# modelstreaming/ams

Hardware: AMD Instinct MI355X
Metric: frames/sec student infer (DeeplabV3+MobileNetV2, 512x1024) + distill-steps/sec (higher is better)
Workload: dtype f32 (2xfp16 split products)

## Files before the change

ams_amd/csrc/k_head.hip:

```cpp
#include "head_common.hpp"

namespace ams {

template <int KMAX>
__global__ __launch_bounds__(256) void upsample_argmax_kernel(const float* __restrict__ logits, HeadGeom g, ClassTable ct,
                                                              const uint8_t* __restrict__ teacher,
                                                              int32_t* __restrict__ labels,
                                                              unsigned long long* __restrict__ conf, double* __restrict__ loss) {
    __shared__ int s_conf[kMaxK * kMaxK];
    __shared__ double s_loss[4];
    __shared__ int s_cnt[4];
    const bool metric = teacher != nullptr;
    if (metric)
        for (int e = threadIdx.x; e < g.K * g.K; e += blockDim.x) s_conf[e] = 0;
    const int b = blockIdx.z;
    if (g.per_frame && metric) { conf += (size_t)b * g.K * g.K; loss += 2 * b; }
    const int x = blockIdx.x * blockDim.x + threadIdx.x;
    if (metric) __syncthreads();
    double my_loss = 0.0;
    int my_cnt = 0;
    int x0 = 0, x1 = 0; float tx = 0.f;
    if (x < g.W) src_tap(x, g.sx, g.w, x0, x1, tx);
    const float* base = logits + (int64_t)b * g.h * g.w * g.ld;
    const int band = (g.H + (int)gridDim.y - 1) / (int)gridDim.y;
    const int ybeg = blockIdx.y * band, yend = ybeg + band < g.H ? ybeg + band : g.H;
    constexpr int KR = KMAX > 0 ? KMAX : 1;
    float top[KR], bot[KR];
    int cur_y0 = -1;
    for (int y = ybeg; y < yend; ++y) {
        if (x >= g.W) break;
        int y0, y1; float ty;
        src_tap(y, g.sy, g.h, y0, y1, ty);
        const float* ptl = base + ((int64_t)y0 * g.w + x0) * g.ld;
        const float* ptr = base + ((int64_t)y0 * g.w + x1) * g.ld;
        const float* pbl = base + ((int64_t)y1 * g.w + x0) * g.ld;
        const float* pbr = base + ((int64_t)y1 * g.w + x1) * g.ld;
        if (KMAX > 0 && y0 != cur_y0) {
            cur_y0 = y0;
#pragma unroll
            for (int k = 0; k < KR; ++k) {
                const int c = ct.idx[k < g.K ? k : 0];
                top[k] = __fadd_rn(ptl[c], __fmul_rn(__fsub_rn(ptr[c], ptl[c]), tx));
                bot[k] = __fadd_rn(pbl[c], __fmul_rn(__fsub_rn(pbr[c], pbl[c]), tx));
            }
        }
        const int64_t pix = ((int64_t)b * g.H + y) * g.W + x;
        int target = -1;
        if (metric) target = ct.lut[teacher[pix]];
        float best = 0.f, zt = 0.f, zmax = 0.f, ssum = 0.f;
        int arg = 0;
        auto visit = [&](int k, float v) {
            if (k == 0 || v > best) { best = v; arg = k; }
            if (target >= 0) {
                if (k == 0) { zmax = v; ssum = 1.f; }
                else if (v > zmax) { ssum = ssum * __expf(zmax - v) + 1.f; zmax = v; }
                else ssum += __expf(v - zmax);
                if (k == target) zt = v;
            }
        };
        if (KMAX > 0) {
#pragma unroll
            for (int k = 0; k < KR; ++k)
                if (k < g.K) visit(k, __fadd_rn(top[k], __fmul_rn(__fsub_rn(bot[k], top[k]), ty)));
        } else {
            for (int k = 0; k < g.K; ++k) {
                const int c = ct.idx[k];
                visit(k, bilerp(ptl[c], ptr[c], pbl[c], pbr[c], tx, ty));
            }
        }
        if (labels) { if (g.labels_u8) reinterpret_cast<uint8_t*>(labels)[pix] = (uint8_t)arg; else labels[pix] = arg; }
        if (target >= 0) {
            my_loss += rint((double)((zmax + __logf(ssum)) - zt) * 1048576.0);
            my_cnt += 1;
            atomicAdd(&s_conf[target * g.K + arg], 1);
        }
    }
    if (!metric) return;
    my_loss = wave_sum(my_loss);
    my_cnt = (int)wave_sum((float)my_cnt);
    const int wave = threadIdx.x >> 6;
    if ((threadIdx.x & 63) == 0) { s_loss[wave] = my_loss; s_cnt[wave] = my_cnt; }
    __syncthreads();
    for (int e = threadIdx.x; e < g.K * g.K; e += blockDim.x)
        if (s_conf[e]) atomicAdd(&conf[e], (unsigned long long)s_conf[e]);
    if (threadIdx.x == 0) {
        const int nw = (blockDim.x + 63) >> 6;
        double ls = 0; int cn = 0;
        for (int i = 0; i < nw; ++i) { ls += s_loss[i]; cn += s_cnt[i]; }
        if (cn) { atomicAdd(&loss[0], ls * (1.0 / 1048576.0)); atomicAdd(&loss[1], (double)cn); }
    }
}

int launch_upsample_argmax(const HeadCall& c, int32_t* labels, int64_t* conf, double* loss, hipStream_t st, int per_frame, int labels_u8) {
    ClassTable ct;
    HeadGeom g;
    if (int rc = head_call_check("upsample_argmax", c, &ct, &g)) return rc;
    AMS_REQUIRE(c.teacher == nullptr || (conf != nullptr && loss != nullptr), "upsample_argmax: metrics need conf and loss buffers");
    AMS_REQUIRE(c.logits, "upsample_argmax: null pointer");
    const int nm = per_frame ? c.B : 1;
    if (c.teacher) {
        AMS_CHECK_HIP(hipMemsetAsync(conf, 0, sizeof(int64_t) * c.K * c.K * nm, st));
        AMS_CHECK_HIP(hipMemsetAsync(loss, 0, sizeof(double) * 2 * nm, st));
    }
    g.per_frame = per_frame;
    g.labels_u8 = labels_u8;
    note_kernel("upsample_argmax_kernel");
    const dim3 grid = head_band_grid(c.B, c.H, c.W);
    if (c.K <= 8)
        hipLaunchKernelGGL(upsample_argmax_kernel<8>, grid, dim3(256), 0, st, c.logits, g, ct, c.teacher, labels, (unsigned long long*)conf, loss);
    else
        hipLaunchKernelGGL(upsample_argmax_kernel<0>, grid, dim3(256), 0, st, c.logits, g, ct, c.teacher, labels, (unsigned long long*)conf, loss);
    AMS_CHECK_LAUNCH();
    return AMS_OK;
}

template <int KMAX>
__global__ __launch_bounds__(256) void ce_grad_kernel(const float* __restrict__ logits, HeadGeom g, ClassTable ct,
                                                      const uint8_t* __restrict__ teacher,
                                                      const double* __restrict__ loss_and_count, float* __restrict__ dlogits,
                                                      int ldd, float empty_val) {
    __shared__ float s_part[4][KMAX];
    const int j = blockIdx.x, i = blockIdx.y, b = blockIdx.z;
    const double nvalid = loss_and_count[1];
    const float inv_n = nvalid > 0.5 ? (float)(1.0 / nvalid) : 0.f;
    const float ry = g.sy > 0.f ? 1.f / g.sy : 0.f, rx = g.sx > 0.f ? 1.f / g.sx : 0.f;
    int ya = g.sy > 0.f ? (int)floorf((i - 1) * ry) - 1 : 0, yb = g.sy > 0.f ? (int)ceilf((i + 1) * ry) + 1 : g.H - 1;
    int xa = g.sx > 0.f ? (int)floorf((j - 1) * rx) - 1 : 0, xb = g.sx > 0.f ? (int)ceilf((j + 1) * rx) + 1 : g.W - 1;
    ya = ya < 0 ? 0 : ya; xa = xa < 0 ? 0 : xa;
    yb = yb > g.H - 1 ? g.H - 1 : yb; xb = xb > g.W - 1 ? g.W - 1 : xb;
    const int ny = yb - ya + 1, nx = xb - xa + 1;
    float acc[KMAX];
#pragma unroll
    for (int k = 0; k < KMAX; ++k) acc[k] = 0.f;
    const float* base = logits + (int64_t)b * g.h * g.w * g.ld;
    for (int p = threadIdx.x; p < ny * nx; p += blockDim.x) {
        const int y = ya + p / nx, x = xa + p % nx;
        int y0, y1, x0, x1; float ty, tx;
        src_tap(y, g.sy, g.h, y0, y1, ty);
        src_tap(x, g.sx, g.w, x0, x1, tx);
        float wy = 0.f, wx = 0.f;
        if (y0 == i) wy += 1.f - ty;
        if (y1 == i) wy += ty;
        if (x0 == j) wx += 1.f - tx;
        if (x1 == j) wx += tx;
        const float wgt = wy * wx;
        if (wgt == 0.f) continue;
        const int target = ct.lut[teacher[((int64_t)b * g.H + y) * g.W + x]];
        if (target < 0) continue;
        const float* ptl = base + ((int64_t)y0 * g.w + x0) * g.ld;
        const float* ptr = base + ((int64_t)y0 * g.w + x1) * g.ld;
        const float* pbl = base + ((int64_t)y1 * g.w + x0) * g.ld;
        const float* pbr = base + ((int64_t)y1 * g.w + x1) * g.ld;
        float z[KMAX];
        float zmax = -3.0e38f;
#pragma unroll
        for (int k = 0; k < KMAX; ++k) {
            if (k < g.K) {
                const int c = ct.idx[k];
                z[k] = bilerp(ptl[c], ptr[c], pbl[c], pbr[c], tx, ty);
                zmax = fmaxf(zmax, z[k]);
            } else z[k] = 0.f;
        }
        float ssum = 0.f;
#pragma unroll
        for (int k = 0; k < KMAX; ++k)
            if (k < g.K) { z[k] = __expf(z[k] - zmax); ssum += z[k]; }
        const float f = wgt * inv_n, rs = 1.f / ssum;
#pragma unroll
        for (int k = 0; k < KMAX; ++k)
            if (k < g.K) acc[k] += f * (z[k] * rs - (k == target ? 1.f : 0.f));
    }
    const int wave = threadIdx.x >> 6, lane = threadIdx.x & 63;
#pragma unroll
    for (int k = 0; k < KMAX; ++k) {
        const float s = wave_sum(acc[k]);
        if (lane == 0) s_part[wave][k] = s;
    }
    __syncthreads();
    float* out = dlogits + (((int64_t)b * g.h + i) * g.w + j) * ldd;
    for (int c = threadIdx.x; c < ldd; c += blockDim.x) {
        float v = 0.f;
        if (c < 256) {
            const int k = ct.lut[c];
            if (k >= 0) v = (s_part[0][k] + s_part[1][k]) + (s_part[2][k] + s_part[3][k]);
            if (k >= 0 && !(nvalid > 0.5)) v = empty_val;
        }
        out[c] = v;
    }
}

int launch_ce_grad(const HeadCall& c, const double* loss_and_count, float* dlogits, int ldd, hipStream_t st, float empty_val) {
    ClassTable ct;
    HeadGeom g;
    if (int rc = head_call_check("ce_grad", c, &ct, &g)) return rc;
    AMS_REQUIRE(ldd >= c.NC && ldd <= 256, "ce_grad: ldd=%d must hold %d classes", ldd, c.NC);
    AMS_REQUIRE(c.logits && c.teacher && loss_and_count && dlogits, "ce_grad: null pointer");
    const dim3 grid(c.w, c.h, c.B);
    note_kernel(c.K <= 8 ? "ce_grad_kernel<8>" : c.K <= 20 ? "ce_grad_kernel<20>" : "ce_grad_kernel<32>");
    if (c.K <= 8)
        hipLaunchKernelGGL(ce_grad_kernel<8>, grid, dim3(256), 0, st, c.logits, g, ct, c.teacher, loss_and_count, dlogits, ldd, empty_val);
    else if (c.K <= 20)
        hipLaunchKernelGGL(ce_grad_kernel<20>, grid, dim3(256), 0, st, c.logits, g, ct, c.teacher, loss_and_count, dlogits, ldd, empty_val);
    else
        hipLaunchKernelGGL(ce_grad_kernel<32>, grid, dim3(256), 0, st, c.logits, g, ct, c.teacher, loss_and_count, dlogits, ldd, empty_val);
    AMS_CHECK_LAUNCH();
    return AMS_OK;
}

constexpr int kCeCB = 10;

template <int KMAX, bool SOFT = false, int KD = 0, bool WT = false>
__global__ __launch_bounds__(192) __attribute__((amdgpu_waves_per_eu(KD != 0 && KMAX == 20 ? 2 : 0)))
void ce_loss_grad_kernel(const float* __restrict__ logits, HeadGeom g, ClassTable ct,
                                                           const uint8_t* __restrict__ teacher, double* __restrict__ loss,
                                                           float* __restrict__ partT, float* __restrict__ partB, SoftTeacher sft, KdParams kd,
                                                           std::conditional_t<WT, LossWeights, NoLossWeights> lw) {
    static_assert(KD == 0 || SOFT, "the KD forms read the teacher logits");
    __shared__ float s_val[192][2 * KMAX + 1];
    __shared__ float s_wx[192][2];
    __shared__ int s_x0[192];
    __shared__ double s_loss[3];
    __shared__ int s_cnt[3];
    __shared__ double s_w[WT ? 3 : 1];
    const int b = blockIdx.z, i0 = blockIdx.y, j_lo = blockIdx.x * kCeCB;
    const int i1 = i0 + 1 < g.h ? i0 + 1 : g.h - 1;
    int ybeg, yend;
    {
        const float inv = g.sy > 0.f ? 1.f / g.sy : 0.f;
        int y = g.sy > 0.f ? (int)(i0 * inv) - 2 : 0;
        if (y < 0) y = 0;
        while (y < g.H && (int)floorf(__fmul_rn((float)y, g.sy)) < i0) ++y;
        ybeg = y;
        while (y < g.H && (int)floorf(__fmul_rn((float)y, g.sy)) == i0) ++y;
        yend = y;
    }
    int xbeg;
    {
        const float inv = g.sx > 0.f ? 1.f / g.sx : 0.f;
        const int jl = j_lo - 1 < 0 ? 0 : j_lo - 1;
        int x = g.sx > 0.f ? (int)(jl * inv) - 2 : 0;
        if (x < 0) x = 0;
        while (x < g.W && (int)floorf(__fmul_rn((float)x, g.sx)) < jl) ++x;
        xbeg = x;
    }
    const int x = xbeg + threadIdx.x;
    int x0 = 0, x1 = 0; float tx = 0.f;
    bool live = x < g.W;
    if (live) { src_tap(x, g.sx, g.w, x0, x1, tx); live = x0 <= j_lo + kCeCB - 1; }
    float gt[KMAX], gb[KMAX];
#pragma unroll
    for (int k = 0; k < KMAX; ++k) { gt[k] = 0.f; gb[k] = 0.f; }
    double my_loss = 0.0;
    int my_cnt = 0;
    [[maybe_unused]] double my_w = 0.0;
    if (live) {
        const float* base = logits + (int64_t)b * g.h * g.w * g.ld;
        const float* ptl = base + ((int64_t)i0 * g.w + x0) * g.ld;
        const float* ptr = base + ((int64_t)i0 * g.w + x1) * g.ld;
        const float* pbl = base + ((int64_t)i1 * g.w + x0) * g.ld;
        const float* pbr = base + ((int64_t)i1 * g.w + x1) * g.ld;
        float top[KMAX], bot[KMAX];
#pragma unroll
        for (int k = 0; k < KMAX; ++k) {
            const int c = ct.idx[k < g.K ? k : 0];
            top[k] = __fadd_rn(ptl[c], __fmul_rn(__fsub_rn(ptr[c], ptl[c]), tx));
            bot[k] = __fadd_rn(pbl[c], __fmul_rn(__fsub_rn(pbr[c], pbl[c]), tx));
        }
        const bool own = x0 >= j_lo;
        int qx0 = 0, qx1 = 0; float qtx = 0.f;
        const float* qbase = nullptr;
        if constexpr (SOFT) {
            src_tap(x, sft.sx, sft.tw, qx0, qx1, qtx);
            qbase = sft.t + (int64_t)b * sft.th * sft.tw * sft.ld;
        }
        const uint8_t* tcol = teacher + (int64_t)b * g.H * g.W + x;
        for (int yb = ybeg; yb < yend; yb += 8) {
          int tgt[8];
#pragma unroll
          for (int r = 0; r < 8; ++r) tgt[r] = tcol[(int64_t)(yb + r < yend ? yb + r : yend - 1) * g.W];
#pragma unroll
          for (int r = 0; r < 8; ++r)
              if constexpr (WT) tgt[r] = (int)lw.pk[tgt[r]];
              else
              tgt[r] = ct.lut[tgt[r]];
#pragma unroll
          for (int r = 0; r < 8; ++r) {
            const int y = yb + r;
            const int target = WT ? (tgt[r] >= 32 ? tgt[r] & 31 : -1) : tgt[r];
            if (y >= yend || target < 0) continue;
            [[maybe_unused]] float wq = 1.f;
            if constexpr (WT) wq = (float)(tgt[r] >> 5) * (1.f / 1048576.f);
            const float src = __fmul_rn((float)y, g.sy);
            const float ty = __fsub_rn(src, floorf(src));
            float z[KMAX];
            float zmax = -3.0e38f, zt = 0.f;
#pragma unroll
            for (int k = 0; k < KMAX; ++k) {
                z[k] = __fadd_rn(top[k], __fmul_rn(__fsub_rn(bot[k], top[k]), ty));
                if (k < g.K) zmax = fmaxf(zmax, z[k]);
                if (k == target) zt = z[k];
            }
            float pt[SOFT ? KMAX : 1];
            float zs[SOFT && KD == 0 ? KMAX : 1];
            if constexpr (SOFT) {
                int qy0, qy1; float qty;
                src_tap(y, sft.sy, sft.th, qy0, qy1, qty);
                const float* qtl = qbase + ((int64_t)qy0 * sft.tw + qx0) * sft.ld;
                float pmax = -3.0e38f;
                if (qty == 0.f && qtx == 0.f) {
#pragma unroll
                    for (int k = 0; k < KMAX; ++k) { pt[k] = qtl[sft.tidx[k < g.K ? k : 0]]; if (k < g.K) pmax = fmaxf(pmax, pt[k]); }
                } else {
                    const float* qtr = qbase + ((int64_t)qy0 * sft.tw + qx1) * sft.ld;
                    const float* qbl = qbase + ((int64_t)qy1 * sft.tw + qx0) * sft.ld;
                    const float* qbr = qbase + ((int64_t)qy1 * sft.tw + qx1) * sft.ld;
#pragma unroll
                    for (int k = 0; k < KMAX; ++k) {
                        const int c = sft.tidx[k < g.K ? k : 0];
                        pt[k] = bilerp(qtl[c], qtr[c], qbl[c], qbr[c], qtx, qty);
                        if (k < g.K) pmax = fmaxf(pmax, pt[k]);
                    }
                }
                float psum = 0.f;
#pragma unroll
                for (int k = 0; k < KMAX; ++k)
                    if constexpr (KD != 0) {
                        const float e = __expf((pt[k] - pmax) * kd.inv_t);
                        pt[k] = k < g.K ? e : 0.f;
                        psum += pt[k];
                    } else {
                    if (k < g.K) { pt[k] = __expf(pt[k] - pmax); psum += pt[k]; } else pt[k] = 0.f;
                    }
                const float rp = 1.f / psum;
#pragma unroll
                for (int k = 0; k < KMAX; ++k) pt[k] *= rp;
                if constexpr (WT) wq = rintf(wq * __expf(-lw.gamma * __logf(psum)) * 1048576.f) * (1.f / 1048576.f);
            }
            if constexpr (KD != 0) {
                float hs[KD == 2 ? KMAX : 1];
                float hard = 0.f;
                if constexpr (KD == 2) {
                    float s1 = 0.f;
#pragma unroll
                    for (int k = 0; k < KMAX; ++k) hs[k] = k < g.K ? __expf(z[k] - zmax) : 0.f;
#pragma unroll
                    for (int k = 0; k < KMAX; ++k) s1 += hs[k];
                    const float r1 = 1.f / s1;
                    hard = (zmax + __logf(s1)) - zt;
#pragma unroll
                    for (int k = 0; k < KMAX; ++k) hs[k] = kd.om * (hs[k] * r1 - (k == target ? 1.f : 0.f));
                }
                float qsum = 0.f, psum1 = 0.f, pz = 0.f;
#pragma unroll
                for (int k = 0; k < KMAX; ++k) {
                    const float zq = (z[k] - zmax) * kd.inv_t;
                    psum1 += pt[k];
                    pz += pt[k] * zq;
                    z[k] = __expf(zq);
                }
#pragma unroll
                for (int k = 0; k < KMAX; ++k) qsum += k < g.K ? z[k] : 0.f;
                const float rq = 1.f / qsum;
                const float lp = __logf(qsum) * psum1 - pz;
                float v = kd.at2 * lp;
                if constexpr (KD == 2) v += kd.om * hard;
                if constexpr (WT) { if (own) { my_loss += rint((double)(wq * v) * 1048576.0); my_w += (double)(wq * 1048576.f); } }
                else
                if (own) { my_loss += rint((double)v * 1048576.0); my_cnt += 1; }
                const float wt = 1.f - ty;
#pragma unroll
                for (int k = 0; k < KMAX; ++k) {
                    float d = kd.at * (z[k] * rq - pt[k]);
                    if constexpr (KD == 2) d += hs[k];
                    if constexpr (WT) d *= wq;
                    gt[k] += wt * d;
                    gb[k] += ty * d;
                }
            } else {
            float ssum = 0.f;
#pragma unroll
            for (int k = 0; k < KMAX; ++k)
                if (k < g.K) { if constexpr (SOFT) zs[k] = z[k] - zmax; z[k] = __expf(z[k] - zmax); ssum += z[k]; }
            const float rs = 1.f / ssum;
            if constexpr (SOFT) {
                const float lse = __logf(ssum);
                float lp = 0.f;
#pragma unroll
                for (int k = 0; k < KMAX; ++k)
                    if (k < g.K) lp += pt[k] * (lse - zs[k]);
                if constexpr (WT) { if (own) { my_loss += rint((double)(wq * lp) * 1048576.0); my_w += (double)(wq * 1048576.f); } }
                else
                if (own) { my_loss += rint((double)lp * 1048576.0); my_cnt += 1; }
            } else {
            if constexpr (WT) { if (own) { my_loss += rint((double)(wq * ((zmax + __logf(ssum)) - zt)) * 1048576.0); my_w += (double)(wq * 1048576.f); } }
            else
            if (own) { my_loss += rint((double)((zmax + __logf(ssum)) - zt) * 1048576.0); my_cnt += 1; }
            }
            const float wt = 1.f - ty;
#pragma unroll
            for (int k = 0; k < KMAX; ++k)
                if (k < g.K) {
                    float want;
                    if constexpr (SOFT) want = pt[k]; else want = k == target ? 1.f : 0.f;
                    float d = z[k] * rs - want;
                    if constexpr (WT) d *= wq;
                    gt[k] += wt * d;
                    gb[k] += ty * d;
                }
            }
          }
        }
    }
#pragma unroll
    for (int k = 0; k < KMAX; ++k) { s_val[threadIdx.x][k] = gt[k]; s_val[threadIdx.x][KMAX + k] = gb[k]; }
    s_x0[threadIdx.x] = live ? x0 : -2;
    s_wx[threadIdx.x][0] = 1.f - tx;
    s_wx[threadIdx.x][1] = x1 != x0 ? tx : 0.f;
    my_loss = wave_sum(my_loss);
    my_cnt = (int)wave_sum((float)my_cnt);
    if constexpr (WT) my_w = wave_sum(my_w);
    if ((threadIdx.x & 63) == 0) { s_loss[threadIdx.x >> 6] = my_loss; s_cnt[threadIdx.x >> 6] = my_cnt; if constexpr (WT) s_w[threadIdx.x >> 6] = my_w; }
    __syncthreads();
    for (int e = threadIdx.x; e < kCeCB * 2 * KMAX; e += blockDim.x) {
        const int jj = e / (2 * KMAX), r = e - jj * (2 * KMAX);
        const int j = j_lo + jj;
        const int tb = r / KMAX, k = r - tb * KMAX;
        if (j >= g.w || k >= g.K) continue;
        float s = 0.f;
        for (int t = 0; t < (int)blockDim.x; ++t) {
            const int c0 = s_x0[t];
            if (c0 == j) s += s_wx[t][0] * s_val[t][r];
            else if (c0 == j - 1) s += s_wx[t][1] * s_val[t][r];
        }
        if (tb == 0) partT[(((int64_t)b * g.h + i0) * g.w + j) * KMAX + k] = s;
        else if (i0 + 1 < g.h) partB[(((int64_t)b * g.h + i0 + 1) * g.w + j) * KMAX + k] = s;
    }
    if (threadIdx.x == 0) {
        double ls = 0; int cn = 0;
        for (int i = 0; i < 3; ++i) { ls += s_loss[i]; cn += s_cnt[i]; }
        double* mine = loss + 2 * (((int64_t)blockIdx.z * gridDim.y + blockIdx.y) * gridDim.x + blockIdx.x);
        mine[0] = ls; mine[1] = (double)cn;
        if constexpr (WT) mine[1] = ((s_w[0] + s_w[1]) + s_w[2]) * (1.0 / 1048576.0);
    }
}

template <int KMAX>
__global__ __launch_bounds__(256) void ce_combine_kernel(const float* __restrict__ partT, const float* __restrict__ partB, int64_t cells,
                                                         int w_cells, int h_cells, ClassTable ct, int K,
                                                         const double* __restrict__ loss_and_count, float* __restrict__ dlogits, int ldd,
                                                         float empty_val) {
    const double nvalid = loss_and_count[1];
    const float inv_n = nvalid > 0 ? (float)(1.0 / nvalid) : 0.f;
    for (int64_t e = blockIdx.x * (int64_t)blockDim.x + threadIdx.x; e < cells * ldd; e += (int64_t)gridDim.x * blockDim.x) {
        const int64_t cell = e / ldd;
        const int c = (int)(e - cell * ldd);
        const int k = c < 256 ? ct.lut[c] : -1;
        float v = 0.f;
        if (k >= 0) {
            const int i = (int)((cell / w_cells) % h_cells);
            const float t = partT[cell * KMAX + k];
            v = (i > 0 ? t + partB[cell * KMAX + k] : t) * inv_n;
            if (!(nvalid > 0)) v = empty_val;
        }
        dlogits[e] = v;
    }
}

bool ce_loss_grad_supported(int w, int W) {
    const int per_cell = w > 1 ? (W - 1 + w - 2) / (w - 1) + 1 : W;
    return (kCeCB + 1) * per_cell + 2 <= 192;
}

size_t ce_loss_grad_scratch(int B, int h, int w, int K) {
    return (size_t)2 * B * h * w * ce_kmax(K) + 4 + (size_t)4 * cdiv(w, kCeCB) * h * B;
}

__global__ __launch_bounds__(256) void ce_loss_sum_kernel(const double* __restrict__ blk, int n, double* __restrict__ loss) {
    __shared__ double s0[4], s1[4];
    double a = 0.0, c = 0.0;
    for (int i = threadIdx.x; i < n; i += 256) { a += blk[2 * (int64_t)i]; c += blk[2 * (int64_t)i + 1]; }
    a = wave_sum(a); c = wave_sum(c);
    if ((threadIdx.x & 63) == 0) { s0[threadIdx.x >> 6] = a; s1[threadIdx.x >> 6] = c; }
    __syncthreads();
    if (threadIdx.x == 0) { loss[0] = ((s0[0] + s0[1]) + (s0[2] + s0[3])) * (1.0 / 1048576.0); loss[1] = (s1[0] + s1[1]) + (s1[2] + s1[3]); }
}

int launch_ce_loss_grad(const HeadCall& c, const LossObjective& o, double* loss, float* scratch, hipStream_t st) {
    if (int rc = kd_params_check("ce_loss_grad", o.temperature, o.alpha)) return rc;
    if (int rc = loss_weights_check("ce_loss_grad", o.class_weights, c.K, c.K, o.conf_gamma)) return rc;
    AMS_REQUIRE(o.conf_gamma == 0.f || o.teacher_logits, "ce_loss_grad: conf_gamma %g weights by the teacher's confidence: it needs teacher logits", (double)o.conf_gamma);
    ClassTable ct;
    HeadGeom g;
    if (int rc = head_call_check("ce_loss_grad", c, &ct, &g)) return rc;
    AMS_REQUIRE(c.logits && c.teacher && loss && scratch, "ce_loss_grad: null pointer");
    AMS_REQUIRE(ce_loss_grad_supported(c.w, c.W), "ce_loss_grad: %d output columns on %d source columns do not fit a block", c.W, c.w);
    const int KM = ce_kmax(c.K);
    const size_t planes = (size_t)2 * c.B * c.h * c.w * KM;
    float* partT = scratch;
    float* partB = scratch + planes / 2;
    const dim3 grid(cdiv(c.w, kCeCB), c.h, c.B);
    double* blk = reinterpret_cast<double*>(scratch + (planes + 3) / 4 * 4);
    SoftTeacher sft;
    memset(&sft, 0, sizeof(sft));
    if (o.teacher_logits) {
        AMS_REQUIRE(o.th >= 1 && o.tw >= 1 && o.th <= c.H && o.tw <= c.W, "ce_loss_grad: teacher logits of %d x %d for labels of %d x %d", o.th, o.tw, c.H, c.W);
        AMS_REQUIRE(tlogits_layout_ok(o.layout), "ce_loss_grad: unknown teacher-logit layout %d", o.layout);
        sft = soft_teacher_geom(o.teacher_logits, o.th, o.tw, o.layout, ct, c.K, c.NC, c.H, c.W);
    }
    KdParams kd;
    kd.inv_t = 1.f / o.temperature;
    kd.at2 = o.alpha * (o.temperature * o.temperature);
    kd.at = o.alpha * o.temperature;
    kd.om = 1.f - o.alpha;
    const LossForm f = loss_form(o, c.K);
    note_kernel(f.name);
    auto launch = [&](auto soft_c, auto kd_c, auto lwv) {
        constexpr bool S = decltype(soft_c)::value, Wt = std::is_same<decltype(lwv), LossWeights>::value;
        constexpr int D = decltype(kd_c)::value;
        if (KM == 8) hipLaunchKernelGGL((ce_loss_grad_kernel<8, S, D, Wt>), grid, dim3(192), 0, st, c.logits, g, ct, c.teacher, blk, partT, partB, sft, kd, lwv);
        else if (KM == 20) hipLaunchKernelGGL((ce_loss_grad_kernel<20, S, D, Wt>), grid, dim3(192), 0, st, c.logits, g, ct, c.teacher, blk, partT, partB, sft, kd, lwv);
        else hipLaunchKernelGGL((ce_loss_grad_kernel<32, S, D, Wt>), grid, dim3(192), 0, st, c.logits, g, ct, c.teacher, blk, partT, partB, sft, kd, lwv);
    };
    auto of_form = [&](auto lwv) {
        using std::bool_constant; using std::integral_constant;
        if (f.kd == 2) launch(bool_constant<true>{}, integral_constant<int, 2>{}, lwv);
        else if (f.kd == 1) launch(bool_constant<true>{}, integral_constant<int, 1>{}, lwv);
        else if (f.soft) launch(bool_constant<true>{}, integral_constant<int, 0>{}, lwv);
        else launch(bool_constant<false>{}, integral_constant<int, 0>{}, lwv);
    };
    if (f.weighted) {
        LossWeights lw;
        fill_loss_weights(ct, o.class_weights, c.K, o.conf_gamma, &lw);
        of_form(lw);
    } else {
        of_form(NoLossWeights{});
    }
    AMS_CHECK_LAUNCH();
    hipLaunchKernelGGL(ce_loss_sum_kernel, dim3(1), dim3(256), 0, st, blk, (int)(grid.x * grid.y * grid.z), loss);
    AMS_CHECK_LAUNCH();
    return AMS_OK;
}

int launch_ce_combine(const HeadCall& c, const double* loss_and_count, const float* scratch, float* dlogits, int ldd, hipStream_t st, float empty_val) {
    ClassTable ct;
    HeadGeom g;
    if (int rc = head_call_check("ce_combine", c, &ct, &g)) return rc;
    AMS_REQUIRE(ldd >= c.NC && ldd <= 256, "ce_combine: ldd=%d must hold %d classes", ldd, c.NC);
    const int KM = ce_kmax(c.K);
    const int64_t cells = (int64_t)c.B * c.h * c.w;
    const float* partT = scratch;
    const float* partB = scratch + (size_t)cells * KM;
    const int grid = (int)(cdiv64(cells * ldd, 256) < 2048 ? cdiv64(cells * ldd, 256) : 2048);
    if (KM == 8) hipLaunchKernelGGL(ce_combine_kernel<8>, dim3(grid), dim3(256), 0, st, partT, partB, cells, c.w, c.h, ct, c.K, loss_and_count, dlogits, ldd, empty_val);
    else if (KM == 20) hipLaunchKernelGGL(ce_combine_kernel<20>, dim3(grid), dim3(256), 0, st, partT, partB, cells, c.w, c.h, ct, c.K, loss_and_count, dlogits, ldd, empty_val);
    else hipLaunchKernelGGL(ce_combine_kernel<32>, dim3(grid), dim3(256), 0, st, partT, partB, cells, c.w, c.h, ct, c.K, loss_and_count, dlogits, ldd, empty_val);
    AMS_CHECK_LAUNCH();
    return AMS_OK;
}

__global__ __launch_bounds__(256) void cross_conf_kernel(const uint8_t* __restrict__ a, const uint8_t* __restrict__ b, int64_t n,
                                                         ClassTable ct, int K, unsigned long long* __restrict__ conf) {
    __shared__ int s_conf[kMaxK * kMaxK];
    cross_conf_block(a, b, n, ct, K, conf, s_conf);
}

int launch_cross_confusion(const uint8_t* a, const uint8_t* b, int64_t n, const int32_t* lut, int K, int64_t* conf,
                           hipStream_t st) {
    AMS_REQUIRE(K > 0 && K <= kMaxK, "cross_confusion: K=%d out of range", K);
    ClassTable ct;
    for (int i = 0; i < 256; ++i) ct.lut[i] = lut[i];
    for (int k = 0; k < kMaxK; ++k) ct.idx[k] = 0;
    AMS_CHECK_HIP(hipMemsetAsync(conf, 0, sizeof(int64_t) * K * K, st));
    int grid = (int)cdiv64(n, 256 * 16);
    if (grid < 1) grid = 1;
    if (grid > 2048) grid = 2048;
    hipLaunchKernelGGL(cross_conf_kernel, dim3(grid), dim3(256), 0, st, a, b, n, ct, K, (unsigned long long*)conf);
    AMS_CHECK_LAUNCH();
    return AMS_OK;
}

}
```

Baseline: 12590.

## Add shared-memory tiled readout kernel with four columns per thread for small K

Adds a readout4 kernel for K<=8 that stages the source logit window for each block into LDS, specialises on K and on metric mode at compile time, and has each thread handle four output columns. Horizontal interpolation results are reused across rows and label stores are vectorised. The aim is to cut redundant global gathers and per-pixel overhead in the upsample-argmax head. The old templated register-caching path is dropped, so the generic kernel becomes the fallback for large K or when the source window does not fit, which may slow that fallback path.

```diff
diff --git a/ams_amd/csrc/k_head.hip b/ams_amd/csrc/k_head.hip
--- a/ams_amd/csrc/k_head.hip
+++ b/ams_amd/csrc/k_head.hip
@@ -2,7 +2,6 @@
 
 namespace ams {
 
-template <int KMAX>
 __global__ __launch_bounds__(256) void upsample_argmax_kernel(const float* __restrict__ logits, HeadGeom g, ClassTable ct,
                                                               const uint8_t* __restrict__ teacher,
                                                               int32_t* __restrict__ labels,
@@ -24,9 +23,6 @@
     const float* base = logits + (int64_t)b * g.h * g.w * g.ld;
     const int band = (g.H + (int)gridDim.y - 1) / (int)gridDim.y;
     const int ybeg = blockIdx.y * band, yend = ybeg + band < g.H ? ybeg + band : g.H;
-    constexpr int KR = KMAX > 0 ? KMAX : 1;
-    float top[KR], bot[KR];
-    int cur_y0 = -1;
     for (int y = ybeg; y < yend; ++y) {
         if (x >= g.W) break;
         int y0, y1; float ty;
@@ -35,15 +31,6 @@
         const float* ptr = base + ((int64_t)y0 * g.w + x1) * g.ld;
         const float* pbl = base + ((int64_t)y1 * g.w + x0) * g.ld;
         const float* pbr = base + ((int64_t)y1 * g.w + x1) * g.ld;
-        if (KMAX > 0 && y0 != cur_y0) {
-            cur_y0 = y0;
-#pragma unroll
-            for (int k = 0; k < KR; ++k) {
-                const int c = ct.idx[k < g.K ? k : 0];
-                top[k] = __fadd_rn(ptl[c], __fmul_rn(__fsub_rn(ptr[c], ptl[c]), tx));
-                bot[k] = __fadd_rn(pbl[c], __fmul_rn(__fsub_rn(pbr[c], pbl[c]), tx));
-            }
-        }
         const int64_t pix = ((int64_t)b * g.H + y) * g.W + x;
         int target = -1;
         if (metric) target = ct.lut[teacher[pix]];
@@ -58,15 +45,9 @@
                 if (k == target) zt = v;
             }
         };
-        if (KMAX > 0) {
-#pragma unroll
-            for (int k = 0; k < KR; ++k)
-                if (k < g.K) visit(k, __fadd_rn(top[k], __fmul_rn(__fsub_rn(bot[k], top[k]), ty)));
-        } else {
-            for (int k = 0; k < g.K; ++k) {
-                const int c = ct.idx[k];
-                visit(k, bilerp(ptl[c], ptr[c], pbl[c], pbr[c], tx, ty));
-            }
+        for (int k = 0; k < g.K; ++k) {
+            const int c = ct.idx[k];
+            visit(k, bilerp(ptl[c], ptr[c], pbl[c], pbr[c], tx, ty));
         }
         if (labels) { if (g.labels_u8) reinterpret_cast<uint8_t*>(labels)[pix] = (uint8_t)arg; else labels[pix] = arg; }
         if (target >= 0) {
@@ -91,6 +72,208 @@
     }
 }
 
+constexpr int kRoCols = 4;
+constexpr int kRoThreads = 256;
+constexpr int kRoBand = 16;
+constexpr int kRoSrcRows = 4;
+constexpr int kRoSrcCols = 128;
+
+__host__ __device__ __forceinline__ void readout4_window(int first, int count, float scale, int n_in, int& lo, int& hi) {
+    const float a = (float)first * scale, b = (float)(first + count - 1) * scale;
+    lo = (int)floorf(a);
+    const int l = (int)floorf(b);
+    hi = l + 1 < n_in ? l + 1 : n_in - 1;
+}
+
+struct RowTap { int y0, y1; float ty; int pad; };
+
+template <int K, bool METRIC>
+__global__ __launch_bounds__(kRoThreads) __attribute__((amdgpu_waves_per_eu(K <= 6 ? 4 : 3))) void readout4_kernel(const float* __restrict__ logits, HeadGeom g, ClassTable ct,
+                                                              const uint8_t* __restrict__ teacher, int32_t* __restrict__ labels,
+                                                              unsigned long long* __restrict__ conf, double* __restrict__ loss, int band, int vec) {
+    __shared__ RowTap s_tap[kRoBand];
+    __shared__ float s_src[kRoSrcRows * kRoSrcCols * K];
+    __shared__ int s_conf[METRIC ? kMaxK * kMaxK : 1];
+    __shared__ double s_loss[METRIC ? 4 : 1];
+    __shared__ int s_cnt[METRIC ? 4 : 1];
+    const int b = blockIdx.z;
+    const int ybeg = blockIdx.y * band;
+    const int nrows = ybeg + band < g.H ? band : g.H - ybeg;
+    if ((int)threadIdx.x < nrows) {
+        RowTap t;
+        src_tap(ybeg + (int)threadIdx.x, g.sy, g.h, t.y0, t.y1, t.ty);
+        t.pad = 0;
+        s_tap[threadIdx.x] = t;
+    }
+    if constexpr (METRIC)
+        for (int e = threadIdx.x; e < K * K; e += blockDim.x) s_conf[e] = 0;
+    const float* base = logits + (int64_t)b * g.h * g.w * g.ld;
+    const int xfirst = blockIdx.x * blockDim.x * kRoCols;
+    const int xlast = xfirst + (int)blockDim.x * kRoCols - 1 < g.W ? xfirst + (int)blockDim.x * kRoCols - 1 : g.W - 1;
+    int ya, yb, xa, xb;
+    readout4_window(ybeg, nrows, g.sy, g.h, ya, yb);
+    readout4_window(xfirst, xlast - xfirst + 1, g.sx, g.w, xa, xb);
+    int nsr = yb - ya + 1, nsc = xb - xa + 1;
+    nsr = nsr < kRoSrcRows ? nsr : kRoSrcRows;
+    nsc = nsc < kRoSrcCols ? nsc : kRoSrcCols;
+    for (int e = threadIdx.x; e < nsc * K; e += blockDim.x) {
+        const int c = e / K, k = e - c * K;
+        for (int r = 0; r < nsr; ++r)
+            s_src[(r * kRoSrcCols + c) * K + k] = base[((ya + r) * g.w + xa + c) * g.ld + ct.idx[k]];
+    }
+    __syncthreads();
+    const int x = (blockIdx.x * blockDim.x + threadIdx.x) * kRoCols;
+    [[maybe_unused]] double my_loss = 0.0;
+    [[maybe_unused]] int my_cnt = 0;
+    if (x < g.W) {
+        unsigned offl[kRoCols], offr[kRoCols];
+        float tx[kRoCols];
+#pragma unroll
+        for (int j = 0; j < kRoCols; ++j) {
+            int x0, x1;
+            src_tap(x + j < g.W ? x + j : g.W - 1, g.sx, g.w, x0, x1, tx[j]);
+            offl[j] = (unsigned)((x0 - xa) * K);
+            offr[j] = (unsigned)((x1 - xa) * K);
+        }
+        const int64_t frame = (int64_t)b * g.H * g.W;
+        float top[kRoCols][K], bot[kRoCols][K], dif[kRoCols][K];
+        auto hrow = [&](int yy, float (&dst)[kRoCols][K]) {
+            const float* row = s_src + (yy - ya) * (kRoSrcCols * K);
+#pragma unroll
+            for (int j = 0; j < kRoCols; ++j)
+#pragma unroll
+                for (int k = 0; k < K; ++k) {
+                    const float l = row[offl[j] + k], r = row[offr[j] + k];
+                    dst[j][k] = __fadd_rn(l, __fmul_rn(__fsub_rn(r, l), tx[j]));
+                }
+        };
+        int cur_y0 = -1, cur_y1 = -1;
+        for (int r = 0; r < nrows; ++r) {
+            const RowTap t = s_tap[r];
+            const int y0 = __builtin_amdgcn_readfirstlane(t.y0), y1 = __builtin_amdgcn_readfirstlane(t.y1);
+            const float ty = t.ty;
+            if (y0 != cur_y0) {
+                if (y0 == cur_y1) {
+#pragma unroll
+                    for (int j = 0; j < kRoCols; ++j)
+#pragma unroll
+                        for (int k = 0; k < K; ++k) top[j][k] = bot[j][k];
+                } else {
+                    hrow(y0, top);
+                }
+                if (y1 != y0) hrow(y1, bot);
+#pragma unroll
+                for (int j = 0; j < kRoCols; ++j)
+#pragma unroll
+                    for (int k = 0; k < K; ++k) {
+                        if (y1 == y0) bot[j][k] = top[j][k];
+                        dif[j][k] = __fsub_rn(bot[j][k], top[j][k]);
+                    }
+                cur_y0 = y0; cur_y1 = y1;
+            }
+            const int pix = (ybeg + r) * g.W + x;
+            int arg[kRoCols];
+#pragma unroll
+            for (int j = 0; j < kRoCols; ++j) {
+                [[maybe_unused]] int target = -1;
+                if constexpr (METRIC)
+                    if (x + j < g.W) target = ct.lut[teacher[frame + pix + j]];
+                float best = 0.f;
+                [[maybe_unused]] float zt = 0.f, zmax = 0.f, ssum = 0.f;
+                int a = 0;
+#pragma unroll
+                for (int k = 0; k < K; ++k) {
+                    const float v = __fadd_rn(top[j][k], __fmul_rn(dif[j][k], ty));
+                    if (k == 0 || v > best) { best = v; a = k; }
+                    if constexpr (METRIC) {
+                        if (target >= 0) {
+                            if (k == 0) { zmax = v; ssum = 1.f; }
+                            else if (v > zmax) { ssum = ssum * __expf(zmax - v) + 1.f; zmax = v; }
+                            else ssum += __expf(v - zmax);
+                            if (k == target) zt = v;
+                        }
+                    }
+                }
+                arg[j] = a;
+                if constexpr (METRIC) {
+                    if (target >= 0) {
+                        my_loss += rint((double)((zmax + __logf(ssum)) - zt) * 1048576.0);
+                        my_cnt += 1;
+                        atomicAdd(&s_conf[target * K + a], 1);
+                    }
+                }
+            }
+            if (labels) {
+                if (g.labels_u8) {
+                    uint8_t* out = reinterpret_cast<uint8_t*>(labels) + frame + pix;
+                    if (vec) *reinterpret_cast<uint32_t*>(out) = (uint32_t)arg[0] | (uint32_t)arg[1] << 8 | (uint32_t)arg[2] << 16 | (uint32_t)arg[3] << 24;
+                    else {
+#pragma unroll
+                        for (int j = 0; j < kRoCols; ++j)
+                            if (x + j < g.W) out[j] = (uint8_t)arg[j];
+                    }
+                } else {
+                    int32_t* out = labels + frame + pix;
+                    if (vec) *reinterpret_cast<int4*>(out) = make_int4(arg[0], arg[1], arg[2], arg[3]);
+                    else {
+#pragma unroll
+                        for (int j = 0; j < kRoCols; ++j)
+                            if (x + j < g.W) out[j] = arg[j];
+                    }
+                }
+            }
+        }
+    }
+    if constexpr (METRIC) {
+        if (g.per_frame) { conf += (size_t)b * K * K; loss += 2 * b; }
+        my_loss = wave_sum(my_loss);
+        my_cnt = (int)wave_sum((float)my_cnt);
+        const int wave = threadIdx.x >> 6;
+        if ((threadIdx.x & 63) == 0) { s_loss[wave] = my_loss; s_cnt[wave] = my_cnt; }
+        __syncthreads();
+        for (int e = threadIdx.x; e < K * K; e += blockDim.x)
+            if (s_conf[e]) atomicAdd(&conf[e], (unsigned long long)s_conf[e]);
+        if (threadIdx.x == 0) {
+            const int nw = (blockDim.x + 63) >> 6;
+            double ls = 0; int cn = 0;
+            for (int i = 0; i < nw; ++i) { ls += s_loss[i]; cn += s_cnt[i]; }
+            if (cn) { atomicAdd(&loss[0], ls * (1.0 / 1048576.0)); atomicAdd(&loss[1], (double)cn); }
+        }
+    }
+}
+
+static int readout4_band(int B, int H, int W) {
+    int band = kRoBand;
+    while (band > 4 && (int64_t)cdiv(W, kRoThreads * kRoCols) * cdiv(H, band) * B < 1024) band /= 2;
+    return band;
+}
+
+static bool readout4_fits(const HeadGeom& g, int band) {
+    for (int y = 0; y < g.H; y += band) {
+        int lo, hi;
+        readout4_window(y, y + band < g.H ? band : g.H - y, g.sy, g.h, lo, hi);
+        if (hi - lo + 1 > kRoSrcRows) return false;
+    }
+    const int cols = kRoThreads * kRoCols;
+    for (int x = 0; x < g.W; x += cols) {
+        int lo, hi;
+        readout4_window(x, x + cols < g.W ? cols : g.W - x, g.sx, g.w, lo, hi);
+        if (hi - lo + 1 > kRoSrcCols) return false;
+    }
+    return true;
+}
+
+template <int K>
+static void launch_readout4(const HeadCall& c, const HeadGeom& g, const ClassTable& ct, int32_t* labels, int64_t* conf, double* loss, hipStream_t st) {
+    const int band = readout4_band(c.B, c.H, c.W);
+    const dim3 grid(cdiv(c.W, kRoThreads * kRoCols), cdiv(c.H, band), c.B);
+    const int vec = c.W % kRoCols == 0 && reinterpret_cast<uintptr_t>(labels) % (g.labels_u8 ? 4 : 16) == 0;
+    if (c.teacher)
+        hipLaunchKernelGGL((readout4_kernel<K, true>), grid, dim3(kRoThreads), 0, st, c.logits, g, ct, c.teacher, labels, (unsigned long long*)conf, loss, band, vec);
+    else
+        hipLaunchKernelGGL((readout4_kernel<K, false>), grid, dim3(kRoThreads), 0, st, c.logits, g, ct, c.teacher, labels, (unsigned long long*)conf, loss, band, vec);
+}
+
 int launch_upsample_argmax(const HeadCall& c, int32_t* labels, int64_t* conf, double* loss, hipStream_t st, int per_frame, int labels_u8) {
     ClassTable ct;
     HeadGeom g;
@@ -104,12 +287,24 @@
     }
     g.per_frame = per_frame;
     g.labels_u8 = labels_u8;
-    note_kernel("upsample_argmax_kernel");
-    const dim3 grid = head_band_grid(c.B, c.H, c.W);
-    if (c.K <= 8)
-        hipLaunchKernelGGL(upsample_argmax_kernel<8>, grid, dim3(256), 0, st, c.logits, g, ct, c.teacher, labels, (unsigned long long*)conf, loss);
-    else
-        hipLaunchKernelGGL(upsample_argmax_kernel<0>, grid, dim3(256), 0, st, c.logits, g, ct, c.teacher, labels, (unsigned long long*)conf, loss);
+    const bool small = (int64_t)c.h * c.w * c.ld < (int64_t)1 << 31 && (int64_t)c.H * c.W + kRoCols < (int64_t)1 << 31 &&
+                       readout4_fits(g, readout4_band(c.B, c.H, c.W));
+    note_kernel(c.K <= 8 && small ? "readout4_kernel" : "upsample_argmax_kernel");
+    if (c.K <= 8 && small) {
+        switch (c.K) {
+            case 1: launch_readout4<1>(c, g, ct, labels, conf, loss, st); break;
+            case 2: launch_readout4<2>(c, g, ct, labels, conf, loss, st); break;
+            case 3: launch_readout4<3>(c, g, ct, labels, conf, loss, st); break;
+            case 4: launch_readout4<4>(c, g, ct, labels, conf, loss, st); break;
+            case 5: launch_readout4<5>(c, g, ct, labels, conf, loss, st); break;
+            case 6: launch_readout4<6>(c, g, ct, labels, conf, loss, st); break;
+            case 7: launch_readout4<7>(c, g, ct, labels, conf, loss, st); break;
+            default: launch_readout4<8>(c, g, ct, labels, conf, loss, st); break;
+        }
+    } else {
+        const dim3 grid = head_band_grid(c.B, c.H, c.W);
+        hipLaunchKernelGGL(upsample_argmax_kernel, grid, dim3(256), 0, st, c.logits, g, ct, c.teacher, labels, (unsigned long long*)conf, loss);
+    }
     AMS_CHECK_LAUNCH();
     return AMS_OK;
 }
```

Result: no change. 12640, median of 6 (+0.4%).
